# givemeone1astkiss/RNA-MPNN

Measured on AMD Instinct MI355X. Metric: nucleotides/sec (forward), k=30 RNA graphs, higher is better.
Workload: dtype bf16; 1 GPU; C2: batch=256 RNAs, n~U[100,140], k=30, default 10-layer RNAMPNN, P=T; max_len=140, weights=closed-form deterministic init (3,536,900 params), parallelism=dp1

## Files before the change

### rna-mpnn_amd/csrc/api.cpp

```cpp
#include "api_internal.h"
#include "kernels_bf16.h"

#include <cstdarg>
#include <cstdlib>
#include <cstdio>
#include <cstring>
#include <string>
#include <vector>

static thread_local char g_err[512] = "";

int fail(int code, const char* fmt, ...) {
    va_list ap;
    va_start(ap, fmt);
    vsnprintf(g_err, sizeof(g_err), fmt, ap);
    va_end(ap);
    return code;
}

extern "C" const char* rnampnn_last_error(void) { return g_err; }
extern "C" const char* rnampnn_version(void) { return "rnampnn-hip 0.1 (gfx950)"; }

static int add_raw(rnampnn_ctx* c, const std::string& key, int64_t numel) {
    RawT t{key, numel, c->raw_floats, false};
// ... 189 lines not shown
        h->prof_ms += ms; h->prof_n += 1;
        h->prof_ms_kind[kind] += ms; h->prof_n_kind[kind] += 1;
    }
    h->ev_used = 0;
    return RNAMPNN_OK;
}
static void profile_reset(rnampnn_handle h) {
    h->prof_ms = 0.0; h->prof_n = 0;
    for (int i = 0; i < 2; ++i) { h->prof_ms_kind[i] = 0.0; h->prof_n_kind[i] = 0; }
}

extern "C" int rnampnn_profile_read(rnampnn_handle h, double* kernel_ms, int64_t* launches, int32_t reset) {
    if (!h) return fail(RNAMPNN_ERR_BAD_ARG, "null handle");
    int rc = profile_collect(h);
    if (rc) return rc;
    if (kernel_ms) *kernel_ms = h->prof_ms;
    if (launches) *launches = h->prof_n;
    if (reset) profile_reset(h);
    return RNAMPNN_OK;
}

extern "C" int rnampnn_profile_read_kinds(rnampnn_handle h, double* kernel_ms2, int64_t* launches2, int32_t reset) {
    if (!h || !kernel_ms2 || !launches2) return fail(RNAMPNN_ERR_BAD_ARG, "rnampnn_profile_read_kinds: null argument");
    int rc = profile_collect(h);
    if (rc) return rc;
    for (int i = 0; i < 2; ++i) { kernel_ms2[i] = h->prof_ms_kind[i]; launches2[i] = h->prof_n_kind[i]; }
    if (reset) profile_reset(h);
    return RNAMPNN_OK;
}

extern "C" int rnampnn_destroy(rnampnn_handle h) {
    if (!h) return RNAMPNN_OK;
    for (auto& e : h->ev) (void)hipEventDestroy(e);
    if (h->raw_arena && !h->raw_external) (void)hipFree(h->raw_arena);
    if (h->der_arena) (void)hipFree(h->der_arena);
    t_wimg_destroy(h->wimg);
    delete h;
    return RNAMPNN_OK;
}

extern "C" int rnampnn_num_weights(rnampnn_handle h) { return h ? (int)h->raw.size() : 0; }

extern "C" int rnampnn_weight_info(rnampnn_handle h, int32_t i, const char** key, int64_t* numel) {
    if (!h || i < 0 || i >= (int)h->raw.size()) return fail(RNAMPNN_ERR_BAD_ARG, "weight index out of range");
    if (key) *key = h->raw[i].key.c_str();
    if (numel) *numel = h->raw[i].numel;
    return RNAMPNN_OK;
}

extern "C" int rnampnn_set_weight(rnampnn_handle h, const char* key, const float* data, int64_t numel,
                                  int32_t is_host, void* stream) {
    if (!h || !key || !data) return fail(RNAMPNN_ERR_BAD_ARG, "rnampnn_set_weight: null argument");
    if (!h->raw_arena) {
        HIP_TRY(hipMalloc((void**)&h->raw_arena, h->raw_floats * sizeof(float)));
        HIP_TRY(hipMemsetAsync(h->raw_arena, 0, h->raw_floats * sizeof(float), (hipStream_t)stream));
    }
    if (!h->der_arena) {
        HIP_TRY(hipMalloc((void**)&h->der_arena, h->der_bytes));
        HIP_TRY(hipMemsetAsync(h->der_arena, 0, h->der_bytes, (hipStream_t)stream));
    }
    for (auto& t : h->raw) {
        if (t.key == key) {
            if (t.numel != numel)
                return fail(RNAMPNN_ERR_WEIGHTS, "weight '%s': expected %lld elements, got %lld", key,
                            (long long)t.numel, (long long)numel);
            HIP_TRY(hipMemcpyAsync(h->raw_arena + t.off, data, (size_t)numel * sizeof(float),
// ... 65 lines not shown
    HIP_TRY(hipMemsetAsync(h->der_arena, 0, h->der_bytes, s));
    finalize_lin(h, h->raw_project, s);
    for (Bert* b : {&h->emb, &h->post}) {
        for (auto& a : b->attn) {
            finalize_lin(h, a.qkv, s); finalize_lin(h, a.out, s);
            if (h->cfg.precision == RNAMPNN_PREC_BF16)
                launch_build_attn_images(rawp(h, a.qkv.w), rawp(h, a.out.w), derp<bf16_t>(h, a.img_qkv), derp<bf16_t>(h, a.img_out), s);
        }
        for (auto& l : b->ffn) finalize_lin(h, l, s);
    }
    for (auto& l : h->edge_embed) finalize_lin(h, l, s);
    for (auto& m : h->mpnn) { finalize_mlp2(h, m.msg, false, s); finalize_mlp2(h, m.edge, true, s); }
    for (auto& l : h->raw_ffn) finalize_lin(h, l, s);
    for (auto& l : h->readout) finalize_lin(h, l, s);
    finalize_chain(h, h->emb.chain, h->emb.ffn, s);
    finalize_chain(h, h->post.chain, h->post.ffn, s);
    finalize_chain(h, h->raw_chain, h->raw_ffn, s);
    finalize_chain(h, h->readout_chain, h->readout, s);
    if (h->cfg.precision == RNAMPNN_PREC_BF16)
        launch_build_embed_image(rawp(h, h->edge_embed[0].w), rawp(h, h->edge_embed[1].w), rawp(h, h->edge_embed[1].b),
                                 derp<bf16_t>(h, h->edge_embed_img), derp<float>(h, h->edge_embed_b1p), s);
    HIP_TRY(hipGetLastError());
    h->finalized = true;
    return RNAMPNN_OK;
}

struct Ws {
    int *len, *cu, *node_b, *nbr;
    float *geom, *geomh, *raw_p, *hA, *hB, *pq_e, *pq_m, *s0, *s1, *n0, *n1, *n2, *logits_p;
    float* coef;
    bf16_t *p_e, *p_m, *q_e, *q_m;
    void* e;
    float* big;
    size_t total;
};

static size_t carve(const rnampnn_ctx* c, int B, size_t Nmax, char* base, Ws* w) {
    size_t off = 0;
    auto take = [&](size_t bytes) { size_t o = off; off += (bytes + 255) / 256 * 256; return base ? base + o : (char*)nullptr; };
    size_t k = c->cfg.num_res_neighbours, F = c->fmax;
    size_t esz = c->cfg.precision == RNAMPNN_PREC_BF16 ? sizeof(bf16_t) : sizeof(float);
    Ws tmp;
    Ws& r = w ? *w : tmp;
    r.len = (int*)take(B * sizeof(int));
    r.cu = (int*)take((B + 1) * sizeof(int));
    r.node_b = (int*)take(Nmax * sizeof(int));
    r.nbr = (int*)take(Nmax * k * sizeof(int));
    r.geom = (float*)take((Nmax + B) * RN_GEOM * sizeof(float));
    r.geomh = (float*)take(c->cfg.precision == RNAMPNN_PREC_BF16 ? (Nmax + B) * RN_GEOMH * sizeof(float) : 0);
    r.raw_p = (float*)take(Nmax * RN_RAWP * sizeof(float));
    r.hA = (float*)take((Nmax + 1) * RN_D * sizeof(float));
    r.hB = (float*)take((Nmax + 1) * RN_D * sizeof(float));
    const bool fastp = c->cfg.precision == RNAMPNN_PREC_BF16;
    r.pq_e = (float*)take(fastp ? (Nmax + 1) * 2 * RN_D * sizeof(float) : (Nmax + 1) * 256 * sizeof(float));
    r.pq_m = (float*)take(fastp ? 0 : (Nmax + 1) * 256 * sizeof(float));
    r.coef = (float*)take((size_t)B * 256 * sizeof(float));
    r.p_e = (bf16_t*)take(fastp ? (Nmax + 1) * RN_D * sizeof(bf16_t) : 0);
    r.p_m = (bf16_t*)take(fastp ? (Nmax + 1) * RN_D * sizeof(bf16_t) : 0);
    r.q_e = (bf16_t*)take(fastp ? (Nmax + 1) * RN_D * sizeof(bf16_t) : 0);
    r.q_m = (bf16_t*)take(fastp ? (Nmax + 1) * RN_D * sizeof(bf16_t) : 0);
    r.s0 = (float*)take(Nmax * F * sizeof(float));
    r.s1 = (float*)take(Nmax * F * sizeof(float));
    r.n0 = (float*)take(Nmax * RN_D * sizeof(float));
    r.n1 = (float*)take(Nmax * RN_D * sizeof(float));
    r.n2 = (float*)take(Nmax * RN_D * sizeof(float));
    r.logits_p = (float*)take(Nmax * 4 * sizeof(float));
    r.e = (void*)take(c->cfg.precision == RNAMPNN_PREC_BF16 ? efrag_bytes((int)Nmax, (int)k) : Nmax * k * RN_D * esz);
    r.big = (float*)take(Nmax * k * RN_D * sizeof(float));
    r.total = off;
    return off;
}

extern "C" size_t rnampnn_workspace_bytes(rnampnn_handle h, int32_t B, int32_t T) {
    if (!h || B <= 0 || T <= 0) return 0;
    return carve(h, B, (size_t)B * T, nullptr, nullptr);
}
extern "C" size_t rnampnn_workspace_bytes_packed(rnampnn_handle h, int32_t B, int32_t N_total) {
    if (!h || B <= 0 || N_total <= 0) return 0;
    return carve(h, B, (size_t)N_total, nullptr, nullptr);
}

struct Run {
    rnampnn_ctx* c;
    PackInfo pk;
    Ws w;
    hipStream_t s;
    bool fast;
    const int* ntot() const { return pk.cu + pk.B; }
};

static void gemm(Run& r, const Lin& l, const float* X, int ldx, float* Y, int ldy, const float* res = nullptr,
                 int ldres = 0, const float* X2 = nullptr, int ldx2 = 0, int K1 = -1) {
    rnampnn_ctx* c = r.c;
    int k1 = K1 < 0 ? l.in_pad : K1;
    int k2 = K1 < 0 ? 0 : l.in_pad - K1;
    if (r.fast && l.out >= 64)
        launch_gemm_bf16(r.ntot(), r.pk.Nmax, X, ldx, k1, X2, ldx2, k2, derp<bf16_t>(c, l.wb), rawp(c, l.b), l.out,
                         l.gelu ? 1 : 0, res, ldres, Y, ldy, r.s, l.h16);
    else
        launch_gemm_f32(r.ntot(), r.pk.Nmax, X, ldx, k1, X2, ldx2, k2, derp<float>(c, l.wt), rawp(c, l.b), l.out,
                        l.gelu ? 1 : 0, res, ldres, Y, ldy, r.s);
}

static bool run_chain(Run& r, const Chain& ch, const std::vector<Lin>& layers, const float* X, int ldx, const float* X2,
                      int ldx2, float* Y, int ldy) {
    if (!r.fast || !ch.ok) return false;
    rnampnn_ctx* c = r.c;
    const float* bias[5] = {nullptr, nullptr, nullptr, nullptr, nullptr};
    for (size_t i = 0; i + 1 < layers.size(); ++i) bias[i] = rawp(c, layers[i].b);
    bias[layers.size() - 1] = derp<float>(c, ch.last_bias);
    return launch_ffn_chain(r.ntot(), r.pk.Nmax, X, ldx, X2, ldx2, ch.K0, ch.H, ch.NH, ch.NOUT, derp<bf16_t>(c, ch.img),
                            bias, Y, ldy, ch.n_valid, r.s) == 0;
}

static int run_bert(Run& r, const Bert& b, float* x, float* out) {
    rnampnn_ctx* c = r.c;
    for (auto& a : b.attn) {
        if (r.fast && launch_attn_layer_rna(r.pk, x, derp<bf16_t>(c, a.img_qkv), rawp(c, a.qkv.b), derp<bf16_t>(c, a.img_out), rawp(c, a.out.b),
                                            b.heads, rawp(c, a.gn_scale), rawp(c, a.gn_shift), c->cfg.padding_len, r.s) == 0)
            continue;
// ... 62 lines not shown
}

static void mpnn_step(Run& r, const Mlp2* we, const Mlp2* wm, const float* h_in, float* h_pre, float* msg_out, bool embed_first = false,
                      int reverse = 0) {
    rnampnn_ctx* c = r.c;
    int k = c->cfg.num_res_neighbours;
    bool timed = c->prof && c->ev_used + 2 <= c->ev.size() && (c->prof_seen++ % c->prof_stride) == 0;
    if (timed) { c->ev_kind[c->ev_used / 2] = (we && wm) ? 0 : 1; (void)hipEventRecord(c->ev[c->ev_used], r.s); }
    if (embed_first) {
        launch_resmpnn_embed_bf16(r.pk, k, r.w.nbr, (bf16_t*)r.w.e, r.w.geomh, derp<bf16_t>(c, c->edge_embed_img), rawp(c, c->edge_embed[0].b),
                                  derp<float>(c, c->edge_embed_b1p), r.w.p_m, r.w.q_m, wbf(c, *wm), h_pre, h_in, reverse, r.s);
    } else if (r.fast) {
        launch_mpnn_bf16(r.pk, k, we != nullptr, wm != nullptr, r.w.nbr, (bf16_t*)r.w.e, r.w.p_e, r.w.q_e, r.w.p_m,
                         r.w.q_m, we ? wbf(c, *we) : MpnnWB{}, wm ? wbf(c, *wm) : MpnnWB{}, h_pre, msg_out, we && we->depth == 1,
                         wm ? h_in : nullptr, reverse, r.s);
    } else {
        MpnnW32 e32 = we ? w32(c, *we) : MpnnW32{}, m32 = wm ? w32(c, *wm) : MpnnW32{};
        launch_mpnn_f32(r.pk, k, we != nullptr, wm != nullptr, r.w.nbr, (float*)r.w.e, r.w.pq_e, r.w.pq_m, e32, m32,
                        h_in, h_pre, msg_out, r.s);
    }
    if (timed) { (void)hipEventRecord(c->ev[c->ev_used + 1], r.s); c->ev_used += 2; }
}

static void unpack_e(Run& r, float* dst) {
    int k = r.c->cfg.num_res_neighbours;
    if (r.fast) {
        launch_efrag_to_rows((const bf16_t*)r.w.e, r.ntot(), r.pk.Nmax, k, r.w.big, r.s);
        launch_unpack_edges(r.pk, k, r.w.big, r.w.nbr, dst, r.s);
    } else {
        launch_unpack_edges(r.pk, k, (const float*)r.w.e, r.w.nbr, dst, r.s);
    }
}

static int begin_run(Run& r, rnampnn_handle h, const float* mask, int B, int T, void* ws, size_t ws_bytes, void* stream,
                     const int32_t* cu_seqlens = nullptr, int n_total = 0) {
    if (!h) return fail(RNAMPNN_ERR_BAD_ARG, "null handle");
    if (!h->finalized) return fail(RNAMPNN_ERR_WEIGHTS, "weights not finalized (call rnampnn_finalize_weights)");
    if ((!mask && !cu_seqlens) || !ws || B <= 0 || T <= 0) return fail(RNAMPNN_ERR_BAD_ARG, "null pointer or non-positive B/T");
    const long long nmax = cu_seqlens ? (long long)n_total : (long long)B * T;
    if (nmax <= 0 || nmax > 0x3fffffffLL / (h->cfg.num_res_neighbours * 4))
        return fail(RNAMPNN_ERR_BAD_ARG, "row count out of range for 32-bit edge indexing; split the batch");
    size_t need = carve(h, B, (size_t)nmax, nullptr, nullptr);
    if (ws_bytes < need) return fail(RNAMPNN_ERR_WORKSPACE, "workspace %zu bytes < required %zu", ws_bytes, need);
    if (((uintptr_t)ws & 255) != 0) return fail(RNAMPNN_ERR_BAD_ARG, "workspace must be 256-byte aligned");
    r.c = h;
    r.s = (hipStream_t)stream;
    r.fast = h->cfg.precision == RNAMPNN_PREC_BF16;
    carve(h, B, (size_t)nmax, (char*)ws, &r.w);
    r.pk.len = r.w.len; r.pk.cu = r.w.cu; r.pk.node_b = r.w.node_b;
    r.pk.B = B; r.pk.T = T; r.pk.Nmax = (int)nmax; r.pk.packed_in = cu_seqlens ? 1 : 0;
    size_t Nmax = r.pk.Nmax;
    ZeroRegions z{};
    auto add = [&](void* p, size_t bytes) { z.ptr[z.n] = p; z.words[z.n] = (unsigned)(bytes / 4); ++z.n; };
    add(r.w.hA + Nmax * RN_D, RN_D * sizeof(float));
    add(r.w.hB + Nmax * RN_D, RN_D * sizeof(float));
    if (r.fast) {
        add(r.w.p_e + Nmax * RN_D, RN_D * sizeof(bf16_t));
        add(r.w.p_m + Nmax * RN_D, RN_D * sizeof(bf16_t));
        add(r.w.q_e + Nmax * RN_D, RN_D * sizeof(bf16_t));
        add(r.w.q_m + Nmax * RN_D, RN_D * sizeof(bf16_t));
    } else {
        add(r.w.pq_e + Nmax * 256, 256 * sizeof(float));
        add(r.w.pq_m + Nmax * 256, 256 * sizeof(float));
    }
    if (cu_seqlens) launch_lengths_from_cu(cu_seqlens, r.pk, r.s);
    else launch_lengths(mask, r.pk, r.s);
    launch_zero_regions(z, r.s);
    return RNAMPNN_OK;
}

struct PackedOut { float* logits; float* embedding; int n_total; };
static int forward_core(Run& r, rnampnn_handle h, const RnaMpnnForwardIO* io, const PackedOut* po);

extern "C" int rnampnn_forward(rnampnn_handle h, const RnaMpnnForwardIO* io, void* ws, size_t ws_bytes, void* stream) {
    if (!io || !io->coords) return fail(RNAMPNN_ERR_BAD_ARG, "rnampnn_forward: null io/coords");
    if (io->stop_after == 0 && !io->logits && !io->embedding)
        return fail(RNAMPNN_ERR_BAD_ARG, "rnampnn_forward: logits (or embedding) output required");
    Run r;
    int rc = begin_run(r, h, io->mask, io->B, io->T, ws, ws_bytes, stream);
    if (rc) return rc;
    return forward_core(r, h, io, nullptr);
}

extern "C" int rnampnn_forward_packed(rnampnn_handle h, const float* coords_packed, const int32_t* cu_seqlens, int32_t B,
                                      int32_t N_total, int32_t T_max, int32_t T_norm, float* logits_packed,
                                      float* embedding_packed, void* ws, size_t ws_bytes, void* stream) {
    if (!coords_packed || !cu_seqlens || (!logits_packed && !embedding_packed))
        return fail(RNAMPNN_ERR_BAD_ARG, "rnampnn_forward_packed: null input or no output");
    Run r;
    int rc = begin_run(r, h, nullptr, B, T_max, ws, ws_bytes, stream, cu_seqlens, N_total);
    if (rc) return rc;
    RnaMpnnForwardIO io;
    memset(&io, 0, sizeof(io));
    io.coords = coords_packed; io.B = B; io.T = T_max; io.T_norm = T_norm;
    PackedOut po{logits_packed, embedding_packed, N_total};
    return forward_core(r, h, &io, &po);
}

static int forward_core(Run& r, rnampnn_handle h, const RnaMpnnForwardIO* io, const PackedOut* po) {
    int rc = RNAMPNN_OK;
    rnampnn_ctx* c = h;
    const RnaMpnnConfig& g = c->cfg;
    if (io->T > g.padding_len)
        return fail(RNAMPNN_ERR_T_GT_P, "max_len %d exceeds padding_len %d", io->T, g.padding_len);
    int k = g.num_res_neighbours, L = g.num_res_mpnn_layers;
    int t_norm = io->T_norm > 0 ? io->T_norm : io->T;
    if (t_norm < io->T) return fail(RNAMPNN_ERR_BAD_ARG, "T_norm %d < T %d", t_norm, io->T);
    Ws& w = r.w;
    hipStream_t s = r.s;

    launch_geom(io->coords, r.pk, t_norm, io->raw, w.raw_p, r.fast ? nullptr : w.geom, r.fast ? w.geomh : nullptr, s);
    const bool fused_first = r.fast && io->stop_after != 1;
    {
        const Lin& l = c->raw_project;
        launch_gemm_f32(r.ntot(), r.pk.Nmax, w.raw_p, RN_RAWP, l.in_pad, nullptr, 0, 0, derp<float>(c, l.wt), rawp(c, l.b), l.out,
                        l.gelu ? 1 : 0, nullptr, 0, w.n0, RN_D, r.s);
    }
    rc = run_bert(r, c->emb, w.n0, w.n1);
    if (!rc) {
        if (fused_first)
            launch_node_update(r.pk, w.n1, rawp(c, c->feat_gn_scale), rawp(c, c->feat_gn_shift), t_norm, w.coef, w.hA, 1,
                               node_job(c, c->mpnn[0].msg, w.p_m, w.q_m), NodeJob{}, r.s);
        else
            launch_graph_norm_packed(r.pk, w.n1, w.hA, rawp(c, c->feat_gn_scale), rawp(c, c->feat_gn_shift), t_norm, r.s);
    }
    if (rc) return rc;
    if (launch_knn(io->coords, r.pk, t_norm, k, w.nbr, io->edge_index, s))
        return fail(RNAMPNN_ERR_UNSUPPORTED, "max_len %d too long for the LDS-resident k-NN row", io->T);
    const bool embed_first = fused_first && L >= 1 && !io->e0 && resmpnn_covers(k, false, false) && !ab_switch("RNAMPNN_EMBED_TWO_LAUNCH");
    if (embed_first) { }
    else if (r.fast)
        launch_edge_embed_bf16(r.pk, k, w.geomh, w.nbr, derp<bf16_t>(c, c->edge_embed_img), rawp(c, c->edge_embed[0].b),
                               derp<float>(c, c->edge_embed_b1p), (bf16_t*)w.e, s);
    else
        launch_edge_embed_f32(r.pk, k, w.geom, w.nbr, derp<float>(c, c->edge_embed[0].wt), rawp(c, c->edge_embed[0].b),
                              g.depth_res_edge_feature > 1 ? derp<float>(c, c->edge_embed[1].wt) : nullptr,
                              g.depth_res_edge_feature > 1 ? rawp(c, c->edge_embed[1].b) : nullptr,
                              g.depth_res_edge_feature, (float*)w.e, s);
    if (io->h0) launch_unpack_nodes(r.pk, w.hA, RN_D, RN_D, io->h0, s);
    if (io->e0) unpack_e(r, io->e0);
    if (io->stop_after == 1) { HIP_TRY(hipGetLastError()); return RNAMPNN_OK; }

    if (!fused_first) node_pq(r, c->mpnn[0].msg, w.hA, false);
    bool edge_pending = false;
    int n_fused = 0;
    for (int l = 0; l < L; ++l) {
        mpnn_step(r, edge_pending ? &c->mpnn[l - 1].edge : nullptr, &c->mpnn[l].msg, w.hA, w.hB, nullptr, l == 0 && embed_first, n_fused++ & 1);
        bool tap_e = io->tap_layer == l + 1 && io->e_layer;
        edge_pending = l + 1 < L;
        const bool need_e = edge_pending || tap_e, need_m = l + 1 < L;
        const float* gsc = rawp(c, c->mpnn[l].gn_scale);
        const float* gsh = rawp(c, c->mpnn[l].gn_shift);
        if (r.fast && (need_e || need_m)) {
            const NodeJob je = need_e ? node_job(c, c->mpnn[l].edge, w.p_e, w.q_e) : NodeJob{};
            const NodeJob jm = need_m ? node_job(c, c->mpnn[l + 1].msg, w.p_m, w.q_m) : NodeJob{};
            launch_node_update(r.pk, w.hB, gsc, gsh, t_norm, w.coef, w.hA, (need_e && need_m) ? 2 : 1, need_e ? je : jm, jm, s);
        } else {
            launch_graph_norm_packed(r.pk, w.hB, w.hA, gsc, gsh, t_norm, s);
            if (need_e) node_pq(r, c->mpnn[l].edge, w.hA, true);
            if (need_m) node_pq(r, c->mpnn[l + 1].msg, w.hA, false);
        }
        if (io->tap_layer == l + 1) {
            if (io->h_layer) launch_unpack_nodes(r.pk, w.hA, RN_D, RN_D, io->h_layer, s);
            if (tap_e) {
                mpnn_step(r, &c->mpnn[l].edge, nullptr, w.hA, w.hB, nullptr, false, n_fused++ & 1);
                edge_pending = false;
                unpack_e(r, io->e_layer);
            }
        }
    }
    float* raw_emb = w.n2;
    rc = run_bert(r, c->post, w.hA, w.n0);
    if (rc) return rc;
    run_ffn(r, c->raw_chain, c->raw_ffn, w.raw_p, RN_RAWP, w.n1);
    launch_graph_norm_packed(r.pk, w.n1, w.n2, rawp(c, c->rawffn_gn_scale), rawp(c, c->rawffn_gn_shift), t_norm, s);
    if (io->h_post) launch_unpack_nodes(r.pk, w.n0, RN_D, RN_D, io->h_post, s);
    if (io->raw_emb) launch_unpack_nodes(r.pk, raw_emb, RN_D, RN_D, io->raw_emb, s);
    if (io->embedding) {
        launch_unpack_nodes_strided(r.pk, w.n0, RN_D, RN_D, io->embedding, 2 * RN_D, 0, s);
        launch_unpack_nodes_strided(r.pk, raw_emb, RN_D, RN_D, io->embedding, 2 * RN_D, RN_D, s);
    }
    if (po && po->embedding) {
        HIP_TRY(hipMemcpy2DAsync(po->embedding, 2 * RN_D * sizeof(float), w.n0, RN_D * sizeof(float), RN_D * sizeof(float),
                                 po->n_total, hipMemcpyDeviceToDevice, s));
        HIP_TRY(hipMemcpy2DAsync(po->embedding + RN_D, 2 * RN_D * sizeof(float), raw_emb, RN_D * sizeof(float),
                                 RN_D * sizeof(float), po->n_total, hipMemcpyDeviceToDevice, s));
    }
    const bool want_logits = io->logits || (po && po->logits);
    float* logits_rows = (po && po->logits) ? po->logits : w.logits_p;
    if (want_logits && run_chain(r, c->readout_chain, c->readout, w.n0, RN_D, raw_emb, RN_D, logits_rows, 4)) {
        if (io->logits) launch_unpack_nodes(r.pk, logits_rows, 4, 4, io->logits, s);
    } else if (want_logits) {
        const float* cur = nullptr;
        int ld = 0;
        float* bufs[2] = {w.s0, w.s1};
        for (size_t i = 0; i < c->readout.size(); ++i) {
            const Lin& l = c->readout[i];
            bool last = i + 1 == c->readout.size();
            float* dst = last ? logits_rows : bufs[i & 1];
            if (i == 0) gemm(r, l, w.n0, RN_D, dst, l.out, nullptr, 0, raw_emb, RN_D, RN_D);
            else gemm(r, l, cur, ld, dst, l.out);
            cur = dst; ld = l.out;
        }
        if (io->logits) launch_unpack_nodes(r.pk, logits_rows, 4, 4, io->logits, s);
    }
    HIP_TRY(hipGetLastError());
    return RNAMPNN_OK;
}
// ... 133 lines not shown
```

### rna-mpnn_amd/csrc/api_internal.h

```cpp
#pragma once
#include "../../include/rnampnn_hip.h"
#include "rnampnn_internal.h"
#include "kernels_train.h"

#include <string>
#include <vector>

__attribute__((visibility("hidden"))) int fail(int code, const char* fmt, ...);
#define HIP_TRY(expr)                                                                      \
    do {                                                                                   \
        hipError_t _e = (expr);                                                            \
        if (_e != hipSuccess) return fail(RNAMPNN_ERR_HIP, "%s: %s", #expr, hipGetErrorString(_e)); \
    } while (0)

__device__ __forceinline__ unsigned long long mix64(unsigned long long x) {
    x ^= x >> 30; x *= 0xBF58476D1CE4E5B9ull; x ^= x >> 27; x *= 0x94D049BB133111EBull; x ^= x >> 31;
    return x;
}

struct RawT {
    std::string key;
    int64_t numel;
    size_t off;
    bool set;
// ... 26 lines not shown
    size_t b2p;
};
struct MpnnLayer { int gn_scale, gn_shift; Mlp2 msg, edge; };

struct rnampnn_ctx {
    RnaMpnnConfig cfg;
    std::vector<RawT> raw;
    size_t raw_floats = 0;
    float* raw_arena = nullptr;
    size_t der_bytes = 0;
    char* der_arena = nullptr;
    bool finalized = false;
    Lin raw_project;
    Bert emb, post;
    int feat_gn_scale, feat_gn_shift;
    std::vector<Lin> edge_embed;
    size_t edge_embed_img = 0;
    size_t edge_embed_b1p = 0;
    std::vector<MpnnLayer> mpnn;
    std::vector<Lin> raw_ffn;
    Chain raw_chain;
    int rawffn_gn_scale, rawffn_gn_shift;
    std::vector<Lin> readout;
    Chain readout_chain;
    int fmax = 0;
    bool prof = false;
    int prof_stride = 1;
    long long prof_seen = 0;
    std::vector<hipEvent_t> ev;
    size_t ev_used = 0;
    std::vector<unsigned char> ev_kind;
    double prof_ms = 0.0, prof_ms_kind[2] = {0.0, 0.0};
    long long prof_n = 0, prof_n_kind[2] = {0, 0};
    struct Tape { int64_t id; int B, T, tnorm; float p; uint64_t seed; const void* ws; bool mixed; const unsigned long long* seed_dev;
                  bool att_mfma; };
    std::vector<Tape> tapes;
    int64_t tape_counter = 0;
    hipEvent_t grad_ev[2] = {nullptr, nullptr};
    const unsigned long long* seed_dev = nullptr;
    WImageCache* wimg = nullptr;
    bool raw_external = false;
};

static inline float* rawp(rnampnn_ctx* c, int idx) { return c->raw_arena + c->raw[idx].off; }
template <typename T> static inline T* derp(rnampnn_ctx* c, size_t off) { return reinterpret_cast<T*>(c->der_arena + off); }
```

### rna-mpnn_amd/csrc/kernels_f32.hip

```cpp
#include "api_internal.h"
#include "bf16_core.h"
#include "graph_norm_dev.h"
#include <cstdlib>

#define WAVE 64
static constexpr float kLEPS = 1.0e6f;

__device__ __forceinline__ float wave_sum(float v) {
#pragma unroll
    for (int o = 32; o > 0; o >>= 1) v += __shfl_xor(v, o, WAVE);
    return v;
}

__global__ void k_lengths(const float* __restrict__ mask, int B, int T, int* __restrict__ len) {
    int b = blockIdx.x;
    float s = 0.f;
    for (int t = threadIdx.x; t < T; t += WAVE) s += mask[(size_t)b * T + t];
    s = wave_sum(s);
    if (threadIdx.x == 0) len[b] = (int)(s + 0.5f);
}

__device__ __forceinline__ int block_exclusive_scan_1024(int v, int* wave_tot , int* total) {
    const int lane = threadIdx.x & 63, wave = threadIdx.x >> 6;
    int inc = v;
#pragma unroll
    for (int o = 1; o < 64; o <<= 1) { const int u = __shfl_up(inc, o, 64); if (lane >= o) inc += u; }
    if (lane == 63) wave_tot[wave] = inc;
    __syncthreads();
    int base = 0, tot = 0;
#pragma unroll
    for (int w = 0; w < 16; ++w) { const int t = wave_tot[w]; if (w < wave) base += t; tot += t; }
    *total = tot;
    return base + inc - v;
// ... 34 lines not shown
    const int g = blockIdx.x;
    if (g >= z.n) return;
    unsigned* p = reinterpret_cast<unsigned*>(z.ptr[g]);
    for (unsigned i = threadIdx.x; i < z.words[g]; i += blockDim.x) p[i] = 0u;
}
__global__ void k_zero_bytes(uint4* __restrict__ p, size_t n16, unsigned char* __restrict__ tail, int ntail) {
    const uint4 z = make_uint4(0u, 0u, 0u, 0u);
    for (size_t i = (size_t)blockIdx.x * blockDim.x + threadIdx.x; i < n16; i += (size_t)gridDim.x * blockDim.x) p[i] = z;
    if (blockIdx.x == 0 && (int)threadIdx.x < ntail) tail[threadIdx.x] = 0;
}
void launch_zero_bytes(void* ptr, size_t bytes, hipStream_t s) {
    if (!bytes) return;
    const size_t n16 = bytes / 16;
    size_t g = (n16 + 255) / 256;
    if (g > 2048) g = 2048;
    if (g < 1) g = 1;
    hipLaunchKernelGGL(k_zero_bytes, dim3((unsigned)g), dim3(256), 0, s, reinterpret_cast<uint4*>(ptr), n16,
                       reinterpret_cast<unsigned char*>(ptr) + n16 * 16, (int)(bytes - n16 * 16));
}
__global__ void k_copy16(const uint4* __restrict__ src, uint4* __restrict__ dst, size_t n16) {
    for (size_t i = (size_t)blockIdx.x * blockDim.x + threadIdx.x; i < n16; i += (size_t)gridDim.x * blockDim.x) dst[i] = src[i];
}
void launch_copy_bytes(void* dst, const void* src, size_t bytes, hipStream_t s) {
    const size_t n16 = bytes / 16;
    if (!n16) return;
    size_t g = (n16 + 255) / 256;
    if (g > 2048) g = 2048;
    hipLaunchKernelGGL(k_copy16, dim3((unsigned)g), dim3(256), 0, s, reinterpret_cast<const uint4*>(src), reinterpret_cast<uint4*>(dst), n16);
}
void launch_zero_regions(const ZeroRegions& z, hipStream_t s) {
    if (z.n > 0) hipLaunchKernelGGL(k_zero_regions, dim3(z.n), dim3(256), 0, s, z);
}

void launch_lengths_from_cu(const int32_t* cu_seqlens, const PackInfo& pk, hipStream_t s) {
    hipLaunchKernelGGL(k_lengths_from_cu, dim3(1), dim3(1024), 0, s, cu_seqlens, pk.B, pk.T, pk.Nmax, pk.len, pk.cu);
}

void launch_lengths(const float* mask, const PackInfo& pk, hipStream_t s) {
    hipLaunchKernelGGL(k_lengths, dim3(pk.B), dim3(WAVE), 0, s, mask, pk.B, pk.T, pk.len);
    hipLaunchKernelGGL(k_scan, dim3(1), dim3(1024), 0, s, pk.len, pk.B, pk.cu);
}

__device__ __forceinline__ void geom_record(const float* c, float* g) {
#pragma unroll
    for (int i = 0; i < 21; ++i) g[i] = c[i];
    float v[5][3];
#pragma unroll
    for (int a = 0; a < 5; ++a) {
#pragma unroll
        for (int d = 0; d < 3; ++d) v[a][d] = c[(a + 1) * 3 + d] - c[a * 3 + d];
        float nr = sqrtf(v[a][0] * v[a][0] + v[a][1] * v[a][1] + v[a][2] * v[a][2]);
        float inv = 1.0f / fmaxf(nr, 1e-12f);
#pragma unroll
        for (int d = 0; d < 3; ++d) g[21 + a * 3 + d] = v[a][d] * inv;
    }
#pragma unroll
    for (int a = 0; a < 4; ++a) {
        float x = v[a][1] * v[a + 1][2] - v[a][2] * v[a + 1][1];
        float y = v[a][2] * v[a + 1][0] - v[a][0] * v[a + 1][2];
        float z = v[a][0] * v[a + 1][1] - v[a][1] * v[a + 1][0];
        float inv = 1.0f / fmaxf(sqrtf(x * x + y * y + z * z), kSEPS);
        g[36 + a * 3 + 0] = x * inv; g[36 + a * 3 + 1] = y * inv; g[36 + a * 3 + 2] = z * inv;
    }
}

__device__ __forceinline__ void geomh_record(const float* g, float* gh) {
#pragma unroll
    for (int i = 0; i < RN_GEOMH; ++i) gh[i] = 0.f;
#pragma unroll
    for (int h = 0; h < 2; ++h) {
#pragma unroll
        for (int a = 0; a < 4; ++a)
            if (4 * h + a < 7)
// ... 82 lines not shown
    float c[21];
    const bool have = !pk.packed_in || t < n;
    const float* src = coords + (size_t)(pk.packed_in ? pk.cu[b] + (t < n ? t : 0) : id) * 21;
#pragma unroll
    for (int i = 0; i < 21; ++i) c[i] = have ? src[i] : 0.f;
    if (t < n) {
        int p = pk.cu[b] + t;
        pk.node_b[p] = b;
        float f[28];
        raw_features(c, f);
        float* rp = raw_p + (size_t)p * RN_RAWP;
#pragma unroll
        for (int i = 0; i < 28; ++i) rp[i] = f[i];
#pragma unroll
        for (int i = 28; i < RN_RAWP; ++i) rp[i] = 0.f;
        if (raw_out) {
            float* ro = raw_out + (size_t)id * RN_RAW;
#pragma unroll
            for (int i = 0; i < 28; ++i) ro[i] = f[i];
        }
        store_geom(c, geom, geomh, (size_t)p);
    } else {
        if (raw_out) {
            float* ro = raw_out + (size_t)id * RN_RAW;
#pragma unroll
            for (int i = 0; i < 21; ++i) ro[i] = kLEPS;
#pragma unroll
            for (int i = 21; i < 28; ++i) ro[i] = 0.f;
        }
        if (t == n) store_geom(c, geom, geomh, (size_t)(pk.Nmax + b));
    }
}

void launch_geom(const float* coords, const PackInfo& pk, int Tp, float* raw_out, float* raw_p, float* geom, float* geomh, hipStream_t s) {
    int total = pk.B * (pk.T + 1);
    hipLaunchKernelGGL(k_geom, dim3((total + 63) / 64), dim3(64), 0, s, coords, pk, Tp, raw_out, raw_p, geom, geomh);
}

template <int G>
__global__ void __launch_bounds__(256) k_knn(const float* __restrict__ coords, PackInfo pk, int Tp, int k, int rows_per_block,
                                              int* __restrict__ nbr, int64_t* __restrict__ eidx) {
    extern __shared__ __attribute__((aligned(16))) float sm[];
    constexpr int GROUPS = 256 / G;
    int b = blockIdx.x;
    int n = pk.len[b];
    int T = pk.T;
    int row0 = blockIdx.y * rows_per_block;
    if (row0 >= T) return;
    int gl = threadIdx.x % G, grp = threadIdx.x / G;
    float* cen = sm;
    float* drow = sm + 3 * T + grp * T;
    if (row0 < n) {
        for (int j = threadIdx.x; j < n; j += 256) {
            const float* c = coords + (size_t)(pk.packed_in ? pk.cu[b] + j : b * T + j) * 21;
            float sx = 0.f, sy = 0.f, sz = 0.f;
#pragma unroll
            for (int a = 0; a < 7; ++a) { sx += c[a * 3]; sy += c[a * 3 + 1]; sz += c[a * 3 + 2]; }
            cen[j * 3] = sx / 7.0f; cen[j * 3 + 1] = sy / 7.0f; cen[j * 3 + 2] = sz / 7.0f;
        }
    }
    __syncthreads();
    int base = pk.cu[b];
    const int row_end = min(T, row0 + rows_per_block);
    for (int i0 = row0; i0 < row_end; i0 += GROUPS) {
        const int i = i0 + grp;
        const bool row_live = i < row_end;
        const bool real = row_live && i < n;
        if (row_live && !real) {
            if (eidx) for (int s = gl; s < k; s += G) eidx[((size_t)b * T + i) * k + s] = -1;
// ... 767 lines not shown
```

### rna-mpnn_amd/csrc/rnampnn_internal.h

```cpp
#pragma once
#include <hip/hip_runtime.h>
#include <stdint.h>
#include <stddef.h>

#define RN_D 128
#define RN_RAW 28
#define RN_RAWP 32
#define RN_ERAW 90
#define RN_ERAWP 96
#define RN_GEOM 48
#define RN_GEOMH 64
#define RN_KMAX 32

typedef unsigned short bf16_t;

#include <mutex>
struct DevAttr { std::mutex mu; size_t have[64] = {}; };
static inline void ensure_dyn_lds(const void* fn, size_t bytes, DevAttr& st) {
    if (bytes <= 64 * 1024) return;
    int dev = 0;
    (void)hipGetDevice(&dev);
    std::lock_guard<std::mutex> g(st.mu);
    size_t& h = st.have[dev & 63];
    if (h < bytes) { (void)hipFuncSetAttribute(fn, hipFuncAttributeMaxDynamicSharedMemorySize, (int)bytes); h = bytes; }
}
#include <stdlib.h>
#include <string.h>
static inline bool ab_switch(const char* name) {
    const char* v = getenv(name);
    return v && strcmp(v, "1") == 0;
}
static inline int rn_num_cus() {
    static int cus[64] = {};
    int dev = 0;
    (void)hipGetDevice(&dev);
    int& n = cus[dev & 63];
    if (!n) {
        hipDeviceProp_t p;
        n = hipGetDeviceProperties(&p, dev) == hipSuccess && p.multiProcessorCount > 0 ? p.multiProcessorCount : 256;
    }
    return n;
}

struct PackInfo {
    int* len;
    int* cu;
    int* node_b;
    int  B, T, Nmax;
    int  packed_in;
};

struct ZeroRegions { void* ptr[8]; unsigned words[8]; int n; };
void launch_zero_regions(const ZeroRegions& z, hipStream_t s);
void launch_zero_bytes(void* ptr, size_t bytes, hipStream_t s);
void launch_copy_bytes(void* dst, const void* src, size_t bytes, hipStream_t s);
void launch_lengths(const float* mask, const PackInfo& pk, hipStream_t s);
void launch_lengths_from_cu(const int32_t* cu_seqlens, const PackInfo& pk, hipStream_t s);
void launch_geom(const float* coords, const PackInfo& pk, int Tp, float* raw_out, float* raw_p, float* geom, float* geomh, hipStream_t s);
int  launch_knn(const float* coords, const PackInfo& pk, int Tp, int k, int* nbr, int64_t* edge_index_out, hipStream_t s);
void launch_edge_embed_f32(const PackInfo& pk, int k, const float* geom, const int* nbr,
                           const float* w0t, const float* b0, const float* w1t, const float* b1, int depth,
                           float* e, hipStream_t s);
struct MpnnW32 {
    const float* wc_t;
    const float* w2_t;
    const float* b2;
    int depth;
};
void launch_mpnn_f32(const PackInfo& pk, int k, bool do_edge, bool do_msg, const int* nbr,
                     float* e, const float* pq_e, const float* pq_m, MpnnW32 we, MpnnW32 wm,
                     const float* h_in, float* h_pre, float* msg_out, hipStream_t s);
void launch_graph_norm_packed(const PackInfo& pk, const float* x, float* y, const float* scale, const float* shift, int t_tot,
                              hipStream_t s);
void launch_graph_norm_padded(const float* x, const float* mask, const float* scale, const float* shift,
                              int B, int T, int t_tot, int D, float* y, hipStream_t s);
void launch_gemm_f32(const int* ntot, int mmax, const float* X, int ldx, int K1, const float* X2, int ldx2, int K2,
                     const float* Wt, const float* bias, int N, int act, const float* res, int ldres,
                     float* Y, int ldy, hipStream_t s);
int  launch_attention_f32(const PackInfo& pk, const float* qkv, int heads, float* out, hipStream_t s);
void launch_unpack_nodes(const PackInfo& pk, const float* src, int ld, int D, float* dst, hipStream_t s);
void launch_unpack_nodes_strided(const PackInfo& pk, const float* src, int ld, int D, float* dst, int dst_ld, int dst_col0, hipStream_t s);
void launch_pack_nodes(const PackInfo& pk, const float* src, int D, float* dst, int ld, hipStream_t s);
void launch_unpack_edges(const PackInfo& pk, int k, const float* src, const int* nbr, float* dst, hipStream_t s);
void launch_pack_edges(const PackInfo& pk, int k, const float* src, float* dst, hipStream_t s);
void launch_pack_index(const PackInfo& pk, int k, const int64_t* edge_index, int* nbr, hipStream_t s);
void launch_transpose(const float* src, int ld_src, int rows, int cols, float* dst, int ld_dst, hipStream_t s);
void launch_argmax_recovery(const float* logits, const float* mask, const int32_t* labels, int B, int T,
                            int8_t* pred, int32_t* correct, int32_t* valid, hipStream_t s);
void launch_sample(const float* logits, const float* mask, int B, int T, float temperature, int n_samples,
                   uint64_t seed, const uint64_t* seed_dev, int8_t* out, hipStream_t s);

// ... 8 lines not shown
```

Measured before the change: 14.18 million nucleotides/s.

## Run k-NN and raw-feature FFN on side streams concurrent with front embedding

Forks two auxiliary HIP streams off the main stream. One runs the zeroing and k-NN search, the other runs the raw-feature FFN plus graph norm, while the main stream runs the raw projection and embedding BERT. Completion events are recorded via hipExtLaunchKernelGGL on the lengths and geom kernels, and the branches are joined before their outputs are used. This aims to fill idle GPU capacity left by small front-end kernels, at the cost of extra streams, events and two new workspace buffers. It falls back to serial execution when the stream is being graph-captured.

Result: no change. 14.26 million nucleotides/s, median of 6 (+0.6%).

```diff
diff --git a/rna-mpnn_amd/csrc/api.cpp b/rna-mpnn_amd/csrc/api.cpp
--- a/rna-mpnn_amd/csrc/api.cpp
+++ b/rna-mpnn_amd/csrc/api.cpp
@@ -245,6 +245,8 @@
 extern "C" int rnampnn_destroy(rnampnn_handle h) {
     if (!h) return RNAMPNN_OK;
     for (auto& e : h->ev) (void)hipEventDestroy(e);
+    for (auto& e : h->br_ev) if (e) (void)hipEventDestroy(e);
+    for (auto& st : h->br_stream) if (st) (void)hipStreamDestroy(st);
     if (h->raw_arena && !h->raw_external) (void)hipFree(h->raw_arena);
     if (h->der_arena) (void)hipFree(h->der_arena);
     t_wimg_destroy(h->wimg);
@@ -376,6 +378,7 @@
     bf16_t *p_e, *p_m, *q_e, *q_m;
     void* e;
     float* big;
+    float* rb0; float* rb1;
     size_t total;
 };
 
@@ -411,6 +414,8 @@
     r.logits_p = (float*)take(Nmax * 4 * sizeof(float));
     r.e = (void*)take(c->cfg.precision == RNAMPNN_PREC_BF16 ? efrag_bytes((int)Nmax, (int)k) : Nmax * k * RN_D * esz);
     r.big = (float*)take(Nmax * k * RN_D * sizeof(float));
+    r.rb0 = (float*)take(Nmax * RN_D * sizeof(float));
+    r.rb1 = (float*)take(Nmax * RN_D * sizeof(float));
     r.total = off;
     return off;
 }
@@ -430,6 +435,8 @@
     Ws w;
     hipStream_t s;
     bool fast;
+    ZeroRegions zero;
+    const float* mask; const int32_t* cu_in;
     const int* ntot() const { return pk.cu + pk.B; }
 };
 
@@ -558,8 +565,13 @@
     }
 }
 
+static void run_lengths(Run& r, hipEvent_t done) {
+    if (r.cu_in) launch_lengths_from_cu(r.cu_in, r.pk, r.s, done);
+    else launch_lengths(r.mask, r.pk, r.s, done);
+}
+
 static int begin_run(Run& r, rnampnn_handle h, const float* mask, int B, int T, void* ws, size_t ws_bytes, void* stream,
-                     const int32_t* cu_seqlens = nullptr, int n_total = 0) {
+                     const int32_t* cu_seqlens = nullptr, int n_total = 0, bool launch = true) {
     if (!h) return fail(RNAMPNN_ERR_BAD_ARG, "null handle");
     if (!h->finalized) return fail(RNAMPNN_ERR_WEIGHTS, "weights not finalized (call rnampnn_finalize_weights)");
     if ((!mask && !cu_seqlens) || !ws || B <= 0 || T <= 0) return fail(RNAMPNN_ERR_BAD_ARG, "null pointer or non-positive B/T");
@@ -576,7 +588,8 @@
     r.pk.len = r.w.len; r.pk.cu = r.w.cu; r.pk.node_b = r.w.node_b;
     r.pk.B = B; r.pk.T = T; r.pk.Nmax = (int)nmax; r.pk.packed_in = cu_seqlens ? 1 : 0;
     size_t Nmax = r.pk.Nmax;
-    ZeroRegions z{};
+    ZeroRegions& z = r.zero;
+    z = ZeroRegions{};
     auto add = [&](void* p, size_t bytes) { z.ptr[z.n] = p; z.words[z.n] = (unsigned)(bytes / 4); ++z.n; };
     add(r.w.hA + Nmax * RN_D, RN_D * sizeof(float));
     add(r.w.hB + Nmax * RN_D, RN_D * sizeof(float));
@@ -589,9 +602,11 @@
         add(r.w.pq_e + Nmax * 256, 256 * sizeof(float));
         add(r.w.pq_m + Nmax * 256, 256 * sizeof(float));
     }
-    if (cu_seqlens) launch_lengths_from_cu(cu_seqlens, r.pk, r.s);
-    else launch_lengths(mask, r.pk, r.s);
-    launch_zero_regions(z, r.s);
+    r.mask = mask; r.cu_in = cu_seqlens;
+    if (launch) {
+        run_lengths(r, nullptr);
+        launch_zero_regions(z, r.s);
+    }
     return RNAMPNN_OK;
 }
 
@@ -603,7 +618,7 @@
     if (io->stop_after == 0 && !io->logits && !io->embedding)
         return fail(RNAMPNN_ERR_BAD_ARG, "rnampnn_forward: logits (or embedding) output required");
     Run r;
-    int rc = begin_run(r, h, io->mask, io->B, io->T, ws, ws_bytes, stream);
+    int rc = begin_run(r, h, io->mask, io->B, io->T, ws, ws_bytes, stream, nullptr, 0, false);
     if (rc) return rc;
     return forward_core(r, h, io, nullptr);
 }
@@ -614,7 +629,7 @@
     if (!coords_packed || !cu_seqlens || (!logits_packed && !embedding_packed))
         return fail(RNAMPNN_ERR_BAD_ARG, "rnampnn_forward_packed: null input or no output");
     Run r;
-    int rc = begin_run(r, h, nullptr, B, T_max, ws, ws_bytes, stream, cu_seqlens, N_total);
+    int rc = begin_run(r, h, nullptr, B, T_max, ws, ws_bytes, stream, cu_seqlens, N_total, false);
     if (rc) return rc;
     RnaMpnnForwardIO io;
     memset(&io, 0, sizeof(io));
@@ -622,6 +637,53 @@
     PackedOut po{logits_packed, embedding_packed, N_total};
     return forward_core(r, h, &io, &po);
 }
+
+#if !defined(RN_EXPERIMENTS) && (defined(RN_EXP_FRONT_SERIAL) || defined(RN_EXP_FRONT_KNN_ONLY) || defined(RN_EXP_RAW_AFTER_EMB))
+#error "the RN_EXP_FRONT_* / RN_EXP_RAW_AFTER_EMB variants of forward_core need -DRN_EXPERIMENTS (tools/build_variant.sh)"
+#endif
+#if defined(RN_EXP_FRONT_KNN_ONLY)
+enum { kForkRaw = -1 };
+#elif defined(RN_EXP_RAW_AFTER_EMB)
+enum { kForkRaw = 2 };
+#else
+enum { kForkRaw = 1 };
+#endif
+
+struct Branches {
+    rnampnn_ctx* c;
+    hipStream_t main;
+    bool on = false;
+    bool forked[2] = {false, false};
+    Branches(rnampnn_ctx* c_, hipStream_t main_) : c(c_), main(main_) {
+#if !defined(RN_EXP_FRONT_SERIAL)
+        hipStreamCaptureStatus st = hipStreamCaptureStatusNone;
+        if (hipStreamIsCapturing(main, &st) != hipSuccess) { (void)hipGetLastError(); return; }
+        if (st != hipStreamCaptureStatusNone) return;
+        if (!c->br_ready) {
+            bool ok = true;
+            for (auto& s : c->br_stream) ok = ok && (s || hipStreamCreateWithFlags(&s, hipStreamNonBlocking) == hipSuccess);
+            for (auto& e : c->br_ev) ok = ok && (e || hipEventCreateWithFlags(&e, hipEventDisableTiming) == hipSuccess);
+            if (!ok) { (void)hipGetLastError(); return; }
+            c->br_ready = true;
+        }
+        on = true;
+#endif
+    }
+    hipEvent_t fork_event(bool forks, int i) const { return forks ? c->br_ev[2 * i] : nullptr; }
+    hipStream_t fork(int i, bool record = false) {
+        if (record) (void)hipEventRecord(c->br_ev[2 * i], main);
+        (void)hipStreamWaitEvent(c->br_stream[i], c->br_ev[2 * i], 0);
+        forked[i] = true;
+        return c->br_stream[i];
+    }
+    void join(int i) {
+        if (!forked[i]) return;
+        (void)hipEventRecord(c->br_ev[2 * i + 1], c->br_stream[i]);
+        (void)hipStreamWaitEvent(main, c->br_ev[2 * i + 1], 0);
+        forked[i] = false;
+    }
+    ~Branches() { join(0); join(1); }
+};
 
 static int forward_core(Run& r, rnampnn_handle h, const RnaMpnnForwardIO* io, const PackedOut* po) {
     int rc = RNAMPNN_OK;
@@ -635,23 +697,44 @@
     Ws& w = r.w;
     hipStream_t s = r.s;
 
-    launch_geom(io->coords, r.pk, t_norm, io->raw, w.raw_p, r.fast ? nullptr : w.geom, r.fast ? w.geomh : nullptr, s);
+    Branches br(c, s);
+    const bool fork_raw = kForkRaw >= 0 && br.on && r.fast && c->raw_chain.ok && io->stop_after != 1;
+    int knn_rc = 0;
+    auto knn_branch = [&](hipStream_t st) {
+        launch_zero_regions(r.zero, st);
+        knn_rc = launch_knn(io->coords, r.pk, t_norm, k, w.nbr, io->edge_index, st);
+    };
+    float* raw_emb = w.rb1;
+    auto raw_branch = [&](hipStream_t st) {
+        Run rb = r;
+        rb.s = st;
+        run_ffn(rb, c->raw_chain, c->raw_ffn, w.raw_p, RN_RAWP, w.rb0);
+        launch_graph_norm_packed(r.pk, w.rb0, raw_emb, rawp(c, c->rawffn_gn_scale), rawp(c, c->rawffn_gn_shift), t_norm, st);
+    };
+    run_lengths(r, br.fork_event(br.on, 0));
+    if (br.on) knn_branch(br.fork(0));
+    else launch_zero_regions(r.zero, s);
+
+    launch_geom(io->coords, r.pk, t_norm, io->raw, w.raw_p, r.fast ? nullptr : w.geom, r.fast ? w.geomh : nullptr, s,
+                br.fork_event(fork_raw && kForkRaw == 1, 1));
     const bool fused_first = r.fast && io->stop_after != 1;
+    if (fork_raw && kForkRaw == 1) raw_branch(br.fork(1));
     {
         const Lin& l = c->raw_project;
         launch_gemm_f32(r.ntot(), r.pk.Nmax, w.raw_p, RN_RAWP, l.in_pad, nullptr, 0, 0, derp<float>(c, l.wt), rawp(c, l.b), l.out,
                         l.gelu ? 1 : 0, nullptr, 0, w.n0, RN_D, r.s);
     }
     rc = run_bert(r, c->emb, w.n0, w.n1);
-    if (!rc) {
-        if (fused_first)
-            launch_node_update(r.pk, w.n1, rawp(c, c->feat_gn_scale), rawp(c, c->feat_gn_shift), t_norm, w.coef, w.hA, 1,
-                               node_job(c, c->mpnn[0].msg, w.p_m, w.q_m), NodeJob{}, r.s);
-        else
-            launch_graph_norm_packed(r.pk, w.n1, w.hA, rawp(c, c->feat_gn_scale), rawp(c, c->feat_gn_shift), t_norm, r.s);
-    }
-    if (rc) return rc;
-    if (launch_knn(io->coords, r.pk, t_norm, k, w.nbr, io->edge_index, s))
+    if (rc) return rc;
+    if (fork_raw && kForkRaw == 2) raw_branch(br.fork(1, true));
+    br.join(0);
+    if (fused_first)
+        launch_node_update(r.pk, w.n1, rawp(c, c->feat_gn_scale), rawp(c, c->feat_gn_shift), t_norm, w.coef, w.hA, 1,
+                           node_job(c, c->mpnn[0].msg, w.p_m, w.q_m), NodeJob{}, r.s);
+    else
+        launch_graph_norm_packed(r.pk, w.n1, w.hA, rawp(c, c->feat_gn_scale), rawp(c, c->feat_gn_shift), t_norm, r.s);
+    if (!br.on) knn_rc = launch_knn(io->coords, r.pk, t_norm, k, w.nbr, io->edge_index, s);
+    if (knn_rc)
         return fail(RNAMPNN_ERR_UNSUPPORTED, "max_len %d too long for the LDS-resident k-NN row", io->T);
     const bool embed_first = fused_first && L >= 1 && !io->e0 && resmpnn_covers(k, false, false) && !ab_switch("RNAMPNN_EMBED_TWO_LAUNCH");
     if (embed_first) { }
@@ -695,11 +778,10 @@
             }
         }
     }
-    float* raw_emb = w.n2;
     rc = run_bert(r, c->post, w.hA, w.n0);
     if (rc) return rc;
-    run_ffn(r, c->raw_chain, c->raw_ffn, w.raw_p, RN_RAWP, w.n1);
-    launch_graph_norm_packed(r.pk, w.n1, w.n2, rawp(c, c->rawffn_gn_scale), rawp(c, c->rawffn_gn_shift), t_norm, s);
+    if (fork_raw) br.join(1);
+    else raw_branch(s);
     if (io->h_post) launch_unpack_nodes(r.pk, w.n0, RN_D, RN_D, io->h_post, s);
     if (io->raw_emb) launch_unpack_nodes(r.pk, raw_emb, RN_D, RN_D, io->raw_emb, s);
     if (io->embedding) {
diff --git a/rna-mpnn_amd/csrc/api_internal.h b/rna-mpnn_amd/csrc/api_internal.h
--- a/rna-mpnn_amd/csrc/api_internal.h
+++ b/rna-mpnn_amd/csrc/api_internal.h
@@ -82,6 +82,9 @@
     std::vector<unsigned char> ev_kind;
     double prof_ms = 0.0, prof_ms_kind[2] = {0.0, 0.0};
     long long prof_n = 0, prof_n_kind[2] = {0, 0};
+    hipStream_t br_stream[2] = {nullptr, nullptr};
+    hipEvent_t br_ev[4] = {nullptr, nullptr, nullptr, nullptr};
+    bool br_ready = false;
     struct Tape { int64_t id; int B, T, tnorm; float p; uint64_t seed; const void* ws; bool mixed; const unsigned long long* seed_dev;
                   bool att_mfma; };
     std::vector<Tape> tapes;
diff --git a/rna-mpnn_amd/csrc/kernels_f32.hip b/rna-mpnn_amd/csrc/kernels_f32.hip
--- a/rna-mpnn_amd/csrc/kernels_f32.hip
+++ b/rna-mpnn_amd/csrc/kernels_f32.hip
@@ -1,4 +1,5 @@
 #include "api_internal.h"
+#include <hip/hip_ext.h>
 #include "bf16_core.h"
 #include "graph_norm_dev.h"
 #include <cstdlib>
@@ -99,13 +100,15 @@
     if (z.n > 0) hipLaunchKernelGGL(k_zero_regions, dim3(z.n), dim3(256), 0, s, z);
 }
 
-void launch_lengths_from_cu(const int32_t* cu_seqlens, const PackInfo& pk, hipStream_t s) {
-    hipLaunchKernelGGL(k_lengths_from_cu, dim3(1), dim3(1024), 0, s, cu_seqlens, pk.B, pk.T, pk.Nmax, pk.len, pk.cu);
-}
-
-void launch_lengths(const float* mask, const PackInfo& pk, hipStream_t s) {
+void launch_lengths_from_cu(const int32_t* cu_seqlens, const PackInfo& pk, hipStream_t s, hipEvent_t done) {
+    if (done) hipExtLaunchKernelGGL(k_lengths_from_cu, dim3(1), dim3(1024), 0, s, nullptr, done, 0, cu_seqlens, pk.B, pk.T, pk.Nmax, pk.len, pk.cu);
+    else hipLaunchKernelGGL(k_lengths_from_cu, dim3(1), dim3(1024), 0, s, cu_seqlens, pk.B, pk.T, pk.Nmax, pk.len, pk.cu);
+}
+
+void launch_lengths(const float* mask, const PackInfo& pk, hipStream_t s, hipEvent_t done) {
     hipLaunchKernelGGL(k_lengths, dim3(pk.B), dim3(WAVE), 0, s, mask, pk.B, pk.T, pk.len);
-    hipLaunchKernelGGL(k_scan, dim3(1), dim3(1024), 0, s, pk.len, pk.B, pk.cu);
+    if (done) hipExtLaunchKernelGGL(k_scan, dim3(1), dim3(1024), 0, s, nullptr, done, 0, (const int*)pk.len, pk.B, pk.cu);
+    else hipLaunchKernelGGL(k_scan, dim3(1), dim3(1024), 0, s, pk.len, pk.B, pk.cu);
 }
 
 __device__ __forceinline__ void geom_record(const float* c, float* g) {
@@ -254,9 +257,11 @@
     }
 }
 
-void launch_geom(const float* coords, const PackInfo& pk, int Tp, float* raw_out, float* raw_p, float* geom, float* geomh, hipStream_t s) {
+void launch_geom(const float* coords, const PackInfo& pk, int Tp, float* raw_out, float* raw_p, float* geom, float* geomh, hipStream_t s,
+                 hipEvent_t done) {
     int total = pk.B * (pk.T + 1);
-    hipLaunchKernelGGL(k_geom, dim3((total + 63) / 64), dim3(64), 0, s, coords, pk, Tp, raw_out, raw_p, geom, geomh);
+    if (done) hipExtLaunchKernelGGL(k_geom, dim3((total + 63) / 64), dim3(64), 0, s, nullptr, done, 0, coords, pk, Tp, raw_out, raw_p, geom, geomh);
+    else hipLaunchKernelGGL(k_geom, dim3((total + 63) / 64), dim3(64), 0, s, coords, pk, Tp, raw_out, raw_p, geom, geomh);
 }
 
 template <int G>
diff --git a/rna-mpnn_amd/csrc/rnampnn_internal.h b/rna-mpnn_amd/csrc/rnampnn_internal.h
--- a/rna-mpnn_amd/csrc/rnampnn_internal.h
+++ b/rna-mpnn_amd/csrc/rnampnn_internal.h
@@ -54,9 +54,10 @@
 void launch_zero_regions(const ZeroRegions& z, hipStream_t s);
 void launch_zero_bytes(void* ptr, size_t bytes, hipStream_t s);
 void launch_copy_bytes(void* dst, const void* src, size_t bytes, hipStream_t s);
-void launch_lengths(const float* mask, const PackInfo& pk, hipStream_t s);
-void launch_lengths_from_cu(const int32_t* cu_seqlens, const PackInfo& pk, hipStream_t s);
-void launch_geom(const float* coords, const PackInfo& pk, int Tp, float* raw_out, float* raw_p, float* geom, float* geomh, hipStream_t s);
+void launch_lengths(const float* mask, const PackInfo& pk, hipStream_t s, hipEvent_t done = nullptr);
+void launch_lengths_from_cu(const int32_t* cu_seqlens, const PackInfo& pk, hipStream_t s, hipEvent_t done = nullptr);
+void launch_geom(const float* coords, const PackInfo& pk, int Tp, float* raw_out, float* raw_p, float* geom, float* geomh, hipStream_t s,
+                 hipEvent_t done = nullptr);
 int  launch_knn(const float* coords, const PackInfo& pk, int Tp, int k, int* nbr, int64_t* edge_index_out, hipStream_t s);
 void launch_edge_embed_f32(const PackInfo& pk, int k, const float* geom, const int* nbr,
                            const float* w0t, const float* b0, const float* w1t, const float* b1, int depth,
```
